# DeepMotionAIResearch/DenseMatchingBenchmark

Measured on AMD Instinct MI355X. Metric: stereo pairs/s (540x960, max_disp=192), higher is better.
Workload: dtype f32; 1 GPU; PSMNet Concatenation-volume + 3D aggregation + soft-argmin, 544x960 (540x960 padded), max_disp=192, batch 4 per GPU; costs_materialised=True, conv3d_mode=exact

## Files before the change

densematchingbenchmark_amd/_lib.py:

```python
import ctypes
import os
import re

import torch

_PKG = os.path.dirname(os.path.abspath(__file__))
DEV_BUILD = os.environ.get("DMB_LIB", "").startswith("dev")
LIB_PATH = os.path.join(_PKG, "lib", "libdmb_hip_%s.so" % os.environ["DMB_LIB"] if DEV_BUILD else "libdmb_hip.so")
DECONV3D_WORKSPACE_BYTES = 2048
CONV_SINGLE_CHAIN = 0x100
DEEPPRUNER_LOSS_WORKSPACE_DOUBLES = 9216
HEADER_PATH = os.path.join(os.path.dirname(_PKG), "include", "dmb_hip.h")

_c_int, _c_float, _c_void_p, _c_ll, _c_double = ctypes.c_int, ctypes.c_float, ctypes.c_void_p, ctypes.c_longlong, ctypes.c_double
_P = _c_void_p
_HI = ctypes.POINTER(ctypes.c_int)
_HF = ctypes.POINTER(ctypes.c_float)

ABI_VERSION = 8

SIGNATURES = {
    "dmb_abi_version": (_c_int, []),
    "dmb_last_error": (ctypes.c_char_p, []),
    "dmb_build_id": (ctypes.c_char_p, []),
    "dmb_cat_fms_f32": (_c_int, [_P, _P, _P, _c_int, _c_int, _c_int, _c_int, _c_int, _HI, _P]),
    "dmb_dif_fms_f32": (_c_int, [_P, _P, _P, _c_int, _c_int, _c_int, _c_int, _c_int, _HI, _P]),
    "dmb_gwc_fms_f32": (_c_int, [_P, _P, _P, _c_int, _c_int, _c_int, _c_int, _c_int, _c_int, _HI, _c_int, _c_int, _P]),
    "dmb_fast_cat_fms_f32": (_c_int, [_P, _P, _P, _P] + [_c_int] * 6 + [_P]),
    "dmb_fast_dif_fms_f32": (_c_int, [_P, _P, _P, _P] + [_c_int] * 7 + [_c_float, _P]),
    "dmb_fast_fms_bwd_f32": (_c_int, [_P] * 9 + [_c_int] * 7 + [_c_float, _P]),
    "dmb_spn_gaterecurrent2d_f32": (_c_int, [_P] * 5 + [_c_int] * 6 + [_P]),
    "dmb_spn_gaterecurrent2d_bwd_f32": (_c_int, [_P] * 10 + [_c_int] * 6 + [_P]),
    "dmb_conv2d_k3_multi_f32": (_c_int, [_c_int, _P, _P, _P, _P, _P, _c_int, _c_int, _c_int, _c_int, _P]),
    "dmb_cat_fms_into_f32": (_c_int, [_P, _P, _P, _c_int, _c_int, _c_int, _c_int, _c_int, _HI, _c_int, _c_int, _P]),
    "dmb_correlation1d_f32": (_c_int, [_P, _P, _P, _c_int, _c_int, _c_int, _c_int, _c_int, _c_float, _P]),
    "dmb_copy_window_f32": (_c_int, [_P, _P, _c_ll, _c_int, _c_int, _c_int, _P]),
    "dmb_catconv_pack_weights_f32": (_c_int, [_P, _P, _c_int, _c_int, _c_int, _c_int, _P]),
    "dmb_catconv_finalize_f32": (_c_int, [_P] * 8 + [_c_int] * 8 + [_P]),
    "dmb_catconv_combine_f32": (_c_int, [_P] * 9 + [_c_int] * 7 + [_P]),
    "dmb_conv3d_packed_floats": (_c_ll, [_c_int, _c_int]),
    "dmb_deconv3d_packed_floats": (_c_ll, [_c_int, _c_int]),
    "dmb_conv3d_pack_weights_f32": (_c_int, [_P, _P, _c_int, _c_int, _P]),
    "dmb_deconv3d_pack_weights_f32": (_c_int, [_P, _P, _c_int, _c_int, _P]),
    "dmb_conv3d_k3_f32": (_c_int, [_P, _P, _P, _P, _P, _P] + [_c_int] * 8 + [_P]),
    "dmb_conv3d_k3_c1_f32": (_c_int, [_P, _P, _c_float, _P, _P] + [_c_int] * 6 + [_P]),
    "dmb_deconv3d_k3s2_f32": (_c_int, [_P, _P, _P, _P, _P, _P] + [_c_int] * 8 + [_P, _P]),
    "dmb_conv3d_k3_hw_f32": (_c_int, [_P, _P, _P, _P, _P, _P] + [_c_int] * 8 + [_P]),
    "dmb_deconv3d_k3_hw_f32": (_c_int, [_P, _P, _P, _P, _P, _P] + [_c_int] * 7 + [_P]),
    "dmb_zero_columns_f32": (_c_int, [_P, _c_ll, _c_int, _c_int, _P]),
    "dmb_trilinear_ac_f32": (_c_int, [_P, _P] + [_c_int] * 7 + [_P]),
    "dmb_deconv3d_k8s4_c1_f32": (_c_int, [_P, _P, _P] + [_c_int] * 4 + [_P]),
    "dmb_deconv3d_k8s4_c1_soft_argmin_f32": (_c_int, [_P, _P, _P, _P] + [_c_int] * 4 + [_c_float, _HF, _P]),
    "dmb_soft_argmin_f32": (_c_int, [_P, _P, _c_int, _c_int, _c_int, _c_int, _c_float, _c_int, _HF, _P]),
    "dmb_soft_argmin_sampled_f32": (_c_int, [_P, _P, _P, _c_int, _c_int, _c_int, _c_int, _c_float, _c_int, _P]),
    "dmb_local_soft_argmin_f32": (_c_int, [_P, _P, _P] + [_c_int] * 8 + [_c_float, _P]),
    "dmb_trilinear_soft_argmin_f32": (_c_int, [_P, _P] + [_c_int] * 7 + [_c_float, _HF, _P]),
    "dmb_trilinear_ac_soft_argmin_f32": (_c_int, [_P, _P, _P] + [_c_int] * 7 + [_c_float, _HF, _P]),
    "dmb_conf_head_packed_floats": (_c_ll, [_c_int, _c_int]),
    "dmb_conf_head_pack_weights_f32": (_c_int, [_P, _P, _c_int, _c_int, _P]),
    "dmb_conf_head_f32": (_c_int, [_P, _P, _P, _P, _P, _P] + [_c_int] * 5 + [_P]),
    "dmb_conf_gather_f32": (_c_int, [_P, _P, _P] + [_c_int] * 4 + [_P]),
    "dmb_conf_phase_conv2d_f32": (_c_int, [_P] * 6 + [_c_int] * 5 + [_P]),
    "dmb_conf_ring_f32": (_c_int, [_P] * 6 + [_c_int] * 5 + [_P]),
    "dmb_conv2d_packed_floats": (_c_ll, [_c_int, _c_int, _c_int]),
    "dmb_conv2d_pack_weights_f32": (_c_int, [_P, _P, _c_int, _c_int, _c_int, _P]),
    "dmb_conv2d_f32": (_c_int, [_P, _P, _P, _P, _P, _P] + [_c_int] * 12 + [_P]),
    "dmb_avgpool2d_f32": (_c_int, [_P, _P] + [_c_int] * 7 + [_P]),
    "dmb_bilinear_ac_f32": (_c_int, [_P, _P] + [_c_int] * 8 + [_P]),
# ... 183 lines not shown
```

densematchingbenchmark_amd/csrc/conv3d.hip:

```cpp
#include <type_traits>

#include "dmb_common.h"

#ifndef DMB_S1_GSTR
#define DMB_S1_GSTR 1
#endif

#ifndef DMB_EPI_LD
#define DMB_EPI_LD 0
#endif
#ifndef DMB_EPI_ST
#define DMB_EPI_ST 0
#endif

namespace dmb {

__global__ void pack_weights_kernel(const float* __restrict__ w, float* __restrict__ wp, int Co, int Ci, int Cipad,
                                    int transposed) {
  const int NTT = cdiv(Co, 32);
  const long long total = (long long)Cipad * 27 * NTT * 32;
  for (long long i = blockIdx.x * (long long)blockDim.x + threadIdx.x; i < total; i += (long long)gridDim.x * blockDim.x) {
    const int lane = (int)(i & 63);
    long long r = i >> 6;
    const int nt = (int)(r % NTT);
// ... 27 lines not shown
    const int nt = (int)(r % NTT);
    r /= NTT;
    const int tap = (int)(r % 27);
    const int kp = (int)(r / 27);
    const int co = nt * 32 + (lane & 31);
    const int ci = 2 * kp + (lane >> 5);
    float v = 0.f;
    if (ci < Ci && co < Co)
      v = transposed == 2 ? jb.w[((size_t)ci * Co + co) * 27 + 26 - tap]
                          : (transposed ? jb.w[((size_t)ci * Co + co) * 27 + tap] : jb.w[((size_t)co * Ci + ci) * 27 + tap]);
    jb.wp[i] = v;
  }
}

struct Affine {
  const float* scale;
  const float* shift;
};

template <int CIN_, int COUT_, int TY_, int TX_, int CK_, int WN_, int SCHED_ = 1, int G_ = 0, int PMIN_ = 0, bool LIN_ = false>
struct S1Cfg {
  static constexpr int CIN = CIN_, COUT = COUT_, TY = TY_, TX = TX_, CK = CK_, WN = WN_, SCHED = SCHED_;
  static constexpr bool LIN = LIN_;
  static constexpr int G = G_;
  static constexpr bool ROWPAIR = G_ != 0;
  static constexpr int GR = G_ ? 32 / G_ : 1;
  static constexpr int WZ = 4 / WN;
  static constexpr int TZ = WZ;
  static constexpr int XOFF = ROWPAIR ? 3 : 0;
  static constexpr int PV = (4 + TX + 1 + 3) / 4 * 4;
  static constexpr int P = ROWPAIR ? (PV > PMIN_ ? PV : PMIN_) : TX + 2;
  static constexpr int ROWS = TY + 2;
  static constexpr int PLANE = ROWS * P;
  static constexpr int ZS = TZ + 2;
  static constexpr int UPR = P / 4, UPC = ZS * ROWS * UPR;
  static constexpr int IPC = (UPC + 63) / 64;
  static constexpr int TR_PITCH = 36;
  static constexpr int XS = ROWPAIR ? TX / (G_ ? G_ : 1) : 1;
  static constexpr int MT = LIN ? 2 : (ROWPAIR ? (TY / GR) * XS : (TY * P + 31) / 32);
  static constexpr int GSTR = (G_ == 16 && TY_ == 4 && !LIN_ && (2 * P) % 32 == 16 && P % 32 != 16 && DMB_S1_GSTR) ? 2 : 1;
  __device__ static constexpr int row_base(int q) { return GSTR == 2 ? q : GR * q; }
  __device__ static constexpr int lane_off(int j) { return ROWPAIR ? (j / (G_ ? G_ : 1)) * GSTR * P + (j % (G_ ? G_ : 1)) : j; }
  __device__ static constexpr int tile_off(int mt) { return ROWPAIR ? row_base(mt / XS) * P + (mt % XS) * G_ : mt * 32; }
  __device__ static void decode(int mt, int j, int& ly, int& lx, bool& valid) {
    if (ROWPAIR) {
      ly = row_base(mt / XS) + GSTR * (j / (G_ ? G_ : 1));
// ... 1 lines not shown
      valid = true;
    } else {
      const int m = mt * 32 + j;
      ly = m / P;
      lx = m - ly * P;
      valid = m < TY * P && lx < TX;
    }
  }
  static constexpr int NTT = COUT / 32;
  static constexpr int NT = NTT / WN;
  static constexpr int CH_STRIDE = ZS * PLANE + (ROWPAIR ? 4 : 36);
  static constexpr int NK = (CK / 2) * 27;
  static constexpr int IN_FLOATS = CK * CH_STRIDE;
  static constexpr int BUF_FLOATS = IN_FLOATS + NK * NTT * 64;
  static constexpr int LDS_FLOATS = 2 * BUF_FLOATS;
  static constexpr int WPE = (ROWPAIR && LDS_FLOATS * 4 * 3 <= 160 * 1024) ? 3 : 2;
  static_assert(ROWPAIR || P <= 64, "one wave stages one tile row per instruction");
  static_assert(CK % 2 == 0 && COUT % (32 * WN) == 0 && IN_FLOATS % 4 == 0, "shape");
  static_assert(!ROWPAIR || LIN || (G_ % 4 == 0 && TX % (G_ ? G_ : 1) == 0 && TY % GR == 0), "row-group tiles need TX % G == 0 and TY % (32 / G) == 0");
  static_assert(!LIN || (ROWPAIR && TY == 3 && TX % 4 == 0 && TX >= 32), "linear tiles: vector path, 3 + 2 staged rows, full-width rows");
  static_assert(!ROWPAIR || ((CK * IPC) % 4 == 0 && NT == 1 && LDS_FLOATS >= 4 * 32 * TR_PITCH), "row-pair staging / scratch");
};

template <int VEC>
__device__ __forceinline__ void store_tile(const f32x16 (&a)[VEC], const float (&sc)[16], const float (&sh)[16],
                                           const float* __restrict__ rb, float* __restrict__ yb, int co0, int h,
                                           unsigned cstride, unsigned o, int relu, int cvalid = 1 << 30) {
  float rv[16][VEC];
  if (rb) {
#pragma unroll
    for (int r = 0; r < 16; ++r) {
      if (co0 + cd_row(r, h) >= cvalid) {
        rv[r][0] = 0.f;
        rv[r][VEC - 1] = 0.f;
        continue;
      }
      const float* rp = rb + (size_t)(co0 + cd_row(r, h)) * cstride + o;
      if (VEC == 2) {
        const float2 t = *reinterpret_cast<const float2*>(rp);
        rv[r][0] = t.x;
        rv[r][VEC - 1] = t.y;
      } else {
        rv[r][0] = *rp;
      }
    }
  }
// ... 12 lines not shown
    if (VEC == 2)
      *reinterpret_cast<float2*>(yp) = make_float2(v[0], v[VEC - 1]);
    else
      *yp = v[0];
  }
}

template <class C, bool WITH_RES, bool STATS = false>
__global__ __launch_bounds__(256, C::WPE) void conv3d_s1_kernel(const float* __restrict__ x, const float* __restrict__ wp,
                                                           const float* __restrict__ scale,
                                                           const float* __restrict__ shift,
                                                           const float* __restrict__ res, float* __restrict__ y, int Ci,
                                                           int D, int H, int W, int ntx, int nty, int ntz, int relu,
                                                           double* __restrict__ stats) {
  extern __shared__ __attribute__((aligned(16))) float lds[];
  const int dbg = DMB_DBG((relu >> 8) & 0xff);
  const int stg = DMB_DBG(relu >> 16);
  relu &= 0xff;
  if (stg > 0 && blockIdx.x < 256u * C::WPE) {
    const int n = (int)(__builtin_amdgcn_s_getreg((3 << 11) | (16 << 6) | 4) & 15u) * stg;
    for (int i = 0; i < n; ++i) __builtin_amdgcn_s_sleep(127);
  }
  int t = xcd_remap(blockIdx.x, gridDim.x);
  const int tx = t % ntx;
  t /= ntx;
  const int ty = t % nty;
  t /= nty;
  const int tz = t % ntz;
  const int b = t / ntz;
  const int p0 = C::LIN ? tx * 64 : 0;
  const int x0 = C::LIN ? 0 : tx * C::TX, y0 = C::LIN ? p0 / W : ty * C::TY, z0 = tz * C::TZ;

  const int wave = __builtin_amdgcn_readfirstlane(threadIdx.x >> 6), lane = threadIdx.x & 63;
  const int j = lane & 31, h = lane >> 5;
  const int wz = wave / C::WN, wn = wave % C::WN;
  const unsigned HW = (unsigned)H * W, DHW = (unsigned)D * HW;
  const float* xb = x + (size_t)b * Ci * DHW;

  f32x16 acc[C::MT][C::NT];

  constexpr int NPL = C::CK * C::ZS;
  static_assert(NPL % 4 == 0, "planes are dealt evenly to the 4 waves");
  constexpr int PPW = NPL / 4;
  constexpr int WCH = C::NK * C::NTT * 64;
  static_assert(WCH % 16 == 0, "weights are staged with 16-byte copies, evenly over 4 waves");
  constexpr int WPW = WCH / 16;
// ... 69 lines not shown
#pragma unroll
    for (int ks = 0; ks < C::NK; ++ks) {
      if (ks + 1 < C::NK) load_frag(ks + 1, af[(ks + 1) & 1], bf[(ks + 1) & 1]);
      if (C::SCHED != 0) __builtin_amdgcn_sched_barrier(0);
#pragma unroll
      for (int mt = 0; mt < C::MT; ++mt)
#pragma unroll
        for (int nt = 0; nt < C::NT; ++nt) {
          if (FIRST && ks == 0) {
            const f32x16 zero = {0.f, 0.f, 0.f, 0.f, 0.f, 0.f, 0.f, 0.f, 0.f, 0.f, 0.f, 0.f, 0.f, 0.f, 0.f, 0.f};
            acc[mt][nt] = DMB_MFMA(af[0][nt], bf[0][mt], zero);
          } else {
            acc[mt][nt] = DMB_MFMA(af[ks & 1][nt], bf[ks & 1][mt], acc[mt][nt]);
          }
        }
      if (C::SCHED != 0) __builtin_amdgcn_sched_barrier(0);
    }
    if (!(dbg & 32)) __syncthreads();
  };
  chunk(std::true_type{}, 0);
  for (int ci = 1; ci < NC; ++ci) chunk(std::false_type{}, ci);

  if (dbg & 1) return;
  const int gz = z0 + wz;
  float* yb = y + (size_t)b * C::COUT * DHW;
  const float* rb = res ? res + (size_t)b * C::COUT * DHW : nullptr;
  if constexpr (C::ROWPAIR) {
    float* my = lds + wave * (32 * C::TR_PITCH);
    const __amdgpu_buffer_rsrc_t yrs = make_rsrc(yb, (unsigned)C::COUT * DHW * 4u);
    const __amdgpu_buffer_rsrc_t rrs = make_rsrc(rb ? rb : yb, (unsigned)C::COUT * DHW * 4u);
    const int px = (lane & 7) * 4;
    const float lo = relu == 1 ? 0.f : -__builtin_inff();
    const float lo2 = relu == 2 ? 0.f : -__builtin_inff();
    float sc4[4], sh4[4];
#pragma unroll
    for (int k = 0; k < 4; ++k) {
      const int co = wn * 32 + k * 8 + (lane >> 3);
      sc4[k] = scale ? scale[co] : 1.f;
      sh4[k] = shift ? shift[co] : 0.f;
    }
    const unsigned kstep = 8u * DHW * 4u;
    auto offset0 = [&](int mt) {
      if constexpr (C::LIN) {
        const unsigned pos = (unsigned)(p0 + mt * 32 + px);
        return (gz < D && pos < HW) ? ((unsigned)(wn * 32 + (lane >> 3)) * DHW + (unsigned)gz * HW + pos) * 4u : DMA_OOB;
      }
// ... 1091 lines not shown
      }
  __syncthreads();
  const int q = wave, oz = q >> 1, oy = q & 1;
  float v[4];
#pragma unroll
  for (int i = 0; i < 4; ++i) {
    float s = tiles[(q * 4 + i) * 64 + lane];
#pragma unroll
    for (int ww = 1; ww < 4; ++ww) s += tiles[ww * C1S_TILE + (q * 4 + i) * 64 + lane];
    v[i] = s + bias;
  }
  const int gx = x0 - 4 + lq * 4, gz = z0 + oz, gy = y0 + 2 * lyp + oy;
  if (lq == 0 || gx >= W || gz >= D || gy >= H) return;
  const size_t o = (size_t)b * DHW + (size_t)gz * HW + (size_t)gy * W + gx;
  float4 r4 = make_float4(v[0], v[1], v[2], v[3]);
  if (res) {
    const float4 r = *reinterpret_cast<const float4*>(res + o);
    r4.x += r.x; r4.y += r.y; r4.z += r.z; r4.w += r.w;
  }
  *reinterpret_cast<float4*>(y + o) = r4;
}


static long long cdiv_ll(long long a, long long b) { return (a + b - 1) / b; }
template <class C>
static int launch_s1(const float* x, const float* wp, const float* scale, const float* shift, const float* res,
                     float* y, int B, int Ci, int D, int H, int W, int relu, hipStream_t st) {
  const int ntx = C::LIN ? cdiv(H * W, 64) : cdiv(W, C::TX), nty = C::LIN ? 1 : cdiv(H, C::TY), ntz = cdiv(D, C::TZ);
  const long long nblk = (long long)B * ntx * nty * ntz;
  if (nblk > 0x7fffffffLL) return fail(DMB_EUNSUPPORTED, "conv3d: grid too large");
  const size_t lds = (size_t)C::LDS_FLOATS * sizeof(float) + (size_t)DMB_OPT(17) * 1024;
  if (DMB_OPT(17)) {
    (void)hipFuncSetAttribute(reinterpret_cast<const void*>(&conv3d_s1_kernel<C, true>), hipFuncAttributeMaxDynamicSharedMemorySize, (int)lds);
    (void)hipFuncSetAttribute(reinterpret_cast<const void*>(&conv3d_s1_kernel<C, false>), hipFuncAttributeMaxDynamicSharedMemorySize, (int)lds);
  }
  if (res) {
    DMB_ENSURE_LDS((&conv3d_s1_kernel<C, true>), (size_t)(lds));
    hipLaunchKernelGGL((conv3d_s1_kernel<C, true>), dim3((unsigned)nblk), dim3(256), lds, st, x, wp, scale, shift, res, y, Ci, D,
                       H, W, ntx, nty, ntz, relu, (double*)nullptr);
  } else {
    DMB_ENSURE_LDS((&conv3d_s1_kernel<C, false>), (size_t)(lds));
    hipLaunchKernelGGL((conv3d_s1_kernel<C, false>), dim3((unsigned)nblk), dim3(256), lds, st, x, wp, scale, shift, res, y, Ci, D,
                       H, W, ntx, nty, ntz, relu, (double*)nullptr);
  }
  return launch_status("conv3d stride-1 launch failed");
}
// ... 242 lines not shown

static bool s1_stats_applicable(const float* x, const float* y, int B, int Ci, int Co, int D, int H, int W) {
  return Co == 32 && Ci > 0 && W % 4 == 0 && (((uintptr_t)x | (uintptr_t)y) & 15) == 0 && (long long)Co * D * H * W * 4 < 0x7fffffffLL &&
         (long long)8 * D * H * W * 4 < 0x7fffffffLL && DMB_OPT(2) == 0;
}
extern "C" long long dmb_conv3d_k3_bnstats_partials(int B, int Ci, int Co, int D, int H, int W) {
  if (B <= 0 || D <= 0 || H <= 0 || W <= 0 || Co != 32 || Ci <= 0 || W % 4 != 0) return 0;
  if ((long long)Co * D * H * W * 4 >= 0x7fffffffLL || (long long)8 * D * H * W * 4 >= 0x7fffffffLL) return 0;
  return s1_blocks32(s1_pick32(B, D, H, W), B, D, H, W);
}
extern "C" int dmb_conv3d_k3_bnstats_f32(const float* x, const float* wpack, float* y, double* stats, int B, int Ci, int Co, int D, int H,
                                         int W, void* stream) {
  if (!x || !wpack || !y || !stats || B <= 0 || Ci <= 0 || D <= 0 || H <= 0 || W <= 0) return fail(DMB_EINVAL, "conv3d_bnstats: bad argument");
  if (!s1_stats_applicable(x, y, B, Ci, Co, D, H, W)) return fail(DMB_EUNSUPPORTED, "conv3d_bnstats: 32 output channels, 16-byte rows");
  hipStream_t st = (hipStream_t)stream;
  switch (s1_pick32(B, D, H, W)) {
    case 0: return launch_s1_stats<S1Cfg<0, 32, 4, 48, 2, 1, 1, 16, 0>>(x, wpack, y, stats, B, Ci, D, H, W, st);
    case 1: return launch_s1_stats<S1Cfg<0, 32, 8, 24, 2, 1, 1, 8, 40>>(x, wpack, y, stats, B, Ci, D, H, W, st);
    case 2: return launch_s1_stats<S1Cfg<0, 32, 4, 32, 2, 1, 1, 16, 0>>(x, wpack, y, stats, B, Ci, D, H, W, st);
    default: return launch_s1_stats<S1Cfg<0, 32, 2, 32, 2, 1, 1, 16, 0>>(x, wpack, y, stats, B, Ci, D, H, W, st);
  }
}

static int dsk_variant(int B, int Ci, int Co, int D, int H, int W) {
  const long long tiles = (long long)B * D * cdiv(H, 2) * cdiv(W, 16);
  const int ncu = num_cus();
  const long long units = tiles * cdiv(Co, 32);
  if (Ci % 8 == 0 && Ci <= 64 && units <= 5LL * ncu) return 3;
  return 0;
}

extern "C" int dmb_deconv3d_k3s2_f32(const float* x, const float* wpack, const float* scale, const float* shift,
                                     const float* residual, float* y, int B, int Ci, int Co, int D, int H, int W, int Wout,
                                     int relu, void* workspace, void* stream) {
  if (!x || !wpack || !y || B <= 0 || Ci <= 0 || D <= 0 || H <= 0 || W <= 0) return fail(DMB_EINVAL, "deconv3d: bad argument");
  if (Wout <= 0 || Wout > 2 * W || Wout <= 2 * W - 8 || (Wout & 1)) return fail(DMB_EINVAL, "deconv3d: Wout must be 2 W, or 2 W minus the (at most 3) doubled padding columns");
  if ((long long)8 * D * H * W * 4 >= 0x7fffffffLL)
    return fail(DMB_EUNSUPPORTED, "deconv3d: 8 input channels of one batch item must stay below 2 GiB (32-bit buffer offsets)");
  hipStream_t st = (hipStream_t)stream;
  const bool single_chain = (relu & DMB_CONV_SINGLE_CHAIN) != 0;
  relu &= 0xff;
  relu |= DMB_OPT(6) << 8;
  {
    int v = single_chain ? 0 : dsk_variant(B, Ci, Co, D, H, W);
    if (DMB_OPT(25) == 1) v = 0;
    if (DMB_OPT(25) >= 2) v = DMB_OPT(25) - 1;
// ... 51 lines not shown
```

densematchingbenchmark_amd/csrc/torch_shim.cpp:

```cpp
#include <torch/extension.h>

#include <c10/hip/HIPStream.h>

#include <string>
#include <tuple>
#include <vector>

#include "dmb_hip.h"

namespace {

PyObject* g_error_class = nullptr;

[[noreturn]] void raise(const std::string& msg) {
  PyErr_SetString(g_error_class ? g_error_class : PyExc_RuntimeError, msg.c_str());
  throw py::error_already_set();
}

void chk(int rc, const char* what) {
  if (rc != DMB_OK) raise(std::string(what) + " failed with code " + std::to_string(rc) + " (" + dmb_last_error() + ")");
}

const at::Tensor& f32(const at::Tensor& t, const char* name) {
  if (!t.is_cuda())
// ... 52 lines not shown
  void* ws = nullptr;
  if (workspace.has_value()) {
    const at::Tensor& w = *workspace;
    if (!w.is_cuda() || w.scalar_type() != at::kInt || !w.is_contiguous() || w.numel() * 4 < DMB_DECONV3D_WORKSPACE_BYTES || w.device() != x.device())
      raise("deconv3d_k3s2: workspace must be a contiguous int32 tensor of DMB_DECONV3D_WORKSPACE_BYTES on the input's device");
    ws = w.data_ptr();
  }
  chk(dmb_deconv3d_k3s2_f32(ptr(x, "x"), ptr(wpack, "wpack"), optr(scale, "scale"), optr(shift, "shift"), optr(residual, "residual"),
                            y.data_ptr<float>(), (int)B, (int)Ci, (int)Co, (int)D, (int)H, (int)W, (int)Wout, (int)relu_flags, ws, stream_of(x)),
      "dmb_deconv3d_k3s2_f32");
  return y;
}

at::Tensor conv3d_k3_c1(const at::Tensor& x, const at::Tensor& w, double bias, const c10::optional<at::Tensor>& residual, int64_t flags) {
  f32(x, "x");
  if (x.dim() != 5) raise("conv3d_k3_c1: x must be [B, Ci, D, H, W]");
  const int64_t B = x.size(0), Ci = x.size(1), D = x.size(2), H = x.size(3), W = x.size(4);
  if (w.numel() != Ci * 27) raise("conv3d_k3_c1: weight does not belong to this channel count");
  at::Tensor y = at::empty({B, 1, D, H, W}, x.options());
  if (residual.has_value() && residual->sizes() != y.sizes()) raise("conv3d_k3_c1 residual: shapes differ");
  chk(dmb_conv3d_k3_c1_f32(ptr(x, "x"), ptr(w, "weight"), (float)bias, optr(residual, "residual"), y.data_ptr<float>(), (int)B, (int)Ci,
                           (int)D, (int)H, (int)W, (int)flags, stream_of(x)),
      "dmb_conv3d_k3_c1_f32");
  return y;
}

std::vector<at::Tensor> trilinear_ac_soft_argmin(const at::Tensor& x, int64_t Do, int64_t Ho, int64_t Wo, double alpha,
                                                 const std::vector<float>& disp_values) {
  f32(x, "x");
  if (x.dim() != 4) raise("trilinear_ac_soft_argmin: x must be [B, D, H, W]");
  if ((int64_t)disp_values.size() != Do) raise("trilinear_ac_soft_argmin: one disparity sample value per output plane");
  const int64_t B = x.size(0);
  at::Tensor y = at::empty({B, Do, Ho, Wo}, x.options()), disp = at::empty({B, 1, Ho, Wo}, x.options());
  chk(dmb_trilinear_ac_soft_argmin_f32(ptr(x, "x"), y.data_ptr<float>(), disp.data_ptr<float>(), (int)B, (int)x.size(1), (int)x.size(2),
                                       (int)x.size(3), (int)Do, (int)Ho, (int)Wo, (float)alpha, disp_values.data(), stream_of(x)),
      "dmb_trilinear_ac_soft_argmin_f32");
  return {y, disp};
}

at::Tensor conv2d(const at::Tensor& x, int64_t coff, int64_t Ci, const at::Tensor& wpack, int64_t Co, int64_t ksize, int64_t stride,
                  int64_t dilation, const c10::optional<at::Tensor>& scale, const c10::optional<at::Tensor>& shift,
                  const c10::optional<at::Tensor>& residual, int64_t res_off, int64_t relu_flags, const c10::optional<at::Tensor>& out,
                  int64_t out_off) {
  f32(x, "x");
  if (x.dim() != 4) raise("conv2d: x must be [B, C, H, W]");
  const int64_t B = x.size(0), Cx = x.size(1), H = x.size(2), W = x.size(3);
// ... 119 lines not shown
}

void set_error_class(py::object cls) {
  Py_XDECREF(g_error_class);
  g_error_class = cls.ptr();
  Py_XINCREF(g_error_class);
}

}

#ifndef DMB_SHIM_ID
#define DMB_SHIM_ID "unknown"
#endif

PYBIND11_MODULE(TORCH_EXTENSION_NAME, m) {
  m.doc() = "thin torch extension over libdmb_hip.so's C ABI (include/dmb_hip.h): unwrap tensors, current HIP stream, raise on error";
  m.def("set_error_class", &set_error_class);
  m.def("build_id", []() { return std::string(DMB_SHIM_ID); });
  m.def("library_build_id", []() { return std::string(dmb_build_id()); });
  m.def("abi_version", []() { return dmb_abi_version(); });
  m.def("conv3d_k3", &conv3d_k3);
  m.def("deconv3d_k3s2", &deconv3d_k3s2);
  m.def("conv3d_k3_c1", &conv3d_k3_c1);
  m.def("trilinear_ac_soft_argmin", &trilinear_ac_soft_argmin);
  m.def("conv2d", &conv2d);
  m.def("copy_window", &copy_window);
  m.def("bn_train_fwd", &bn_train_fwd);
  m.def("bn_act_bwd", &bn_act_bwd);
  m.def("conv2d_wgrad", &conv2d_wgrad);
}
```

densematchingbenchmark_amd/modeling/stereo/cost_processors/aggregators/PSMNet.py:

```python
import torch
import torch.nn as nn

from ..... import ops
from ...layers import train_fn
from ...layers.basic_layers import HeadConv3d, conv3d_bn, conv3d_bn_relu
from ..utils.hourglass import Hourglass


class PSMAggregator(nn.Module):

    accepts_lazy_cat = True

    def __init__(self, max_disp, in_planes=64, batch_norm=True):
        super().__init__()
        self.max_disp, self.in_planes, self.batch_norm = max_disp, in_planes, batch_norm
        bn = batch_norm
        self.dres0 = nn.Sequential(conv3d_bn_relu(bn, in_planes, 32, 3, 1, 1, bias=False),
                                   conv3d_bn_relu(bn, 32, 32, 3, 1, 1, bias=False))
        self.dres1 = nn.Sequential(conv3d_bn_relu(bn, 32, 32, 3, 1, 1, bias=False),
                                   conv3d_bn(bn, 32, 32, 3, 1, 1, bias=False))
        self.dres2 = Hourglass(in_planes=32, batch_norm=bn)
        self.dres3 = Hourglass(in_planes=32, batch_norm=bn)
        self.dres4 = Hourglass(in_planes=32, batch_norm=bn)
        self.classif1 = nn.Sequential(conv3d_bn_relu(bn, 32, 32, 3, 1, 1, bias=False), HeadConv3d(32, bias=False))
        self.classif2 = nn.Sequential(conv3d_bn_relu(bn, 32, 32, 3, 1, 1, bias=False), HeadConv3d(32, bias=False))
        self.classif3 = nn.Sequential(conv3d_bn_relu(bn, 32, 32, 3, 1, 1, bias=False), HeadConv3d(32, bias=False))

    def trunk(self, raw_cost):
        cost0 = self.dres0(raw_cost)
        cost0 = self.dres1[1](self.dres1[0](cost0), residual=cost0)
        out1, pre1, post1 = self.dres2(cost0, None, None, skip=cost0)
        out2, pre2, post2 = self.dres3(out1, pre1, post1, skip=cost0)
        out3, pre3, post3 = self.dres4(out2, pre2, post2, skip=cost0)
        cost1 = self.classif1[1](self.classif1[0](out1))
        cost2 = self.classif2[1](self.classif2[0](out2), residual=cost1)
        cost3 = self.classif3[1](self.classif3[0](out3), residual=cost2)
        return cost1, cost2, cost3

    def _forward_overlapped(self, raw_cost):
        B, C, D, H, W = raw_cost.shape
        size = (self.max_disp, H * 4, W * 4)
        vals = ops.disp_sample_values(self.max_disp, 0, 1)
        main = torch.cuda.current_stream(raw_cost.device)
        side = ops.side_stream(raw_cost.device)

        def upsample(c):
            cost, disp = ops.trilinear_ac_soft_argmin(c.squeeze(1), size, vals, 1.0)
            cost.record_stream(main)
            disp.record_stream(main)
            return ops.RegressionHint.attach(cost, vals, 1.0, disp)

        cost0 = self.dres0(raw_cost)
        cost0 = self.dres1[1](self.dres1[0](cost0), residual=cost0)
        out1, pre1, post1 = self.dres2(cost0, None, None, skip=cost0)
        fork1 = main.record_event()
        with torch.cuda.stream(side):
            side.wait_event(fork1)
            cost1 = self.classif1[1](self.classif1[0](out1))
            up1 = upsample(cost1)
        out2, pre2, post2 = self.dres3(out1, pre1, post1, skip=cost0)
        fork2 = main.record_event()
        with torch.cuda.stream(side):
            side.wait_event(fork2)
            cost2 = self.classif2[1](self.classif2[0](out2), residual=cost1)
            cost2.record_stream(main)
            join2 = side.record_event()
            up2 = upsample(cost2)
            done = side.record_event()
        out3, pre3, post3 = self.dres4(out2, pre2, post2, skip=cost0)
        main.wait_event(join2)
        cost3 = self.classif3[1](self.classif3[0](out3), residual=cost2)
        up3 = upsample(cost3)
        main.wait_event(done)
        return [up3, up2, up1]

    def forward(self, raw_cost):
        B, C, D, H, W = raw_cost.shape
        if ops.branch_overlap(raw_cost) and raw_cost.device.type == "cuda" and not train_fn.wants_grad(self, raw_cost):
            return self._forward_overlapped(raw_cost)
        with train_fn.carry_scope():
            cost1, cost2, cost3 = self.trunk(raw_cost)
        size = (self.max_disp, H * 4, W * 4)
        vals = ops.disp_sample_values(self.max_disp, 0, 1)
        up = []
        for c in (cost3, cost2, cost1):
            if train_fn.wants_grad(self, c):
                cost, disp = train_fn.UpsampleRegressFn.apply(c.squeeze(1), size, tuple(vals), 1.0)
            else:
                cost, disp = ops.trilinear_ac_soft_argmin(c.squeeze(1), size, vals, 1.0)
            up.append(ops.RegressionHint.attach(cost, vals, 1.0, disp))
        return up
```

densematchingbenchmark_amd/modeling/stereo/layers/basic_layers.py:

```python
import torch
import torch.nn as nn

from .... import ops, param_state
from . import train_fn

__all__ = ["FusedConv3d", "HeadConv3d", "HeadDeconv3d", "conv3d_bn", "conv3d_bn_relu", "deconv3d_bn", "deconv3d_bn_relu",
           "bn_parts", "fold_batch_norm"]


def fold_batch_norm(bn, conv_bias, out_planes, device):
    if bn is None:
        if conv_bias is None:
            return None, None
        return torch.ones(out_planes, dtype=torch.float32, device=device), conv_bias.detach().float().contiguous()
    if bn.running_mean is None or bn.running_var is None:
        raise NotImplementedError("fold_batch_norm: a BatchNorm without running statistics (track_running_stats=False) "
                                  "normalises with batch statistics in eval() too; it has no folded form")
    var = bn.running_var.detach().double()
    mean = bn.running_mean.detach().double()
    gamma = bn.weight.detach().double() if bn.affine else torch.ones_like(var)
    beta = bn.bias.detach().double() if bn.affine else torch.zeros_like(var)
    scale = gamma / torch.sqrt(var + bn.eps)
    shift = beta - mean * scale
    if conv_bias is not None:
        shift = shift + conv_bias.detach().double() * scale
    return scale.float().contiguous(), shift.float().contiguous()


def bn_parts(bn):
    return () if bn is None else (bn.weight, bn.bias, bn.running_mean, bn.running_var, bn.num_batches_tracked)
# ... 123 lines not shown

class HeadConv3d(nn.Conv3d):

    def __init__(self, in_planes, bias=False):
        super().__init__(in_planes, 1, kernel_size=3, stride=1, padding=1, bias=bias)

    def train(self, mode=True):
        epoch_on_mode_switch(self, mode)
        return super().train(mode)

    def forward(self, x, residual=None):
        if hasattr(x, "materialize"):
            x = x.materialize()
        if train_fn.wants_grad(self, x, residual):
            return train_fn.HeadConvFn.apply(x, self.weight, self.bias, residual)
        return ops.conv3d_k3_c1(x, self.weight.detach(), self.bias_value(), residual)

    def bias_value(self):
        if self.bias is None:
            return 0.0
        return param_state.cached(self, "_dmb_bias", (self.bias,), lambda: float(self.bias.detach().cpu()[0]))


class HeadDeconv3d(nn.ConvTranspose3d):

    def __init__(self, in_planes, out_planes):
        super().__init__(in_planes, out_planes, kernel_size=3, stride=2, padding=1, output_padding=1)

    def forward(self, x):
        if train_fn.wants_grad(self, x):
            return train_fn.HeadDeconvFn.apply(x, self.weight, self.bias)
        wp, bias = param_state.cached(self, "_dmb_packed", (self.weight, self.bias), lambda: (
            ops.pack_deconv3d_weights(self.weight.detach()), self.bias.detach().float().contiguous()))
        return ops.deconv3d_k3s2(x, wp, self.out_channels, None, bias, None, False)


def conv3d_bn(batchNorm, in_planes, out_planes, kernel_size=3, stride=1, padding=1, dilation=1, bias=True):
    return FusedConv3d(batchNorm, in_planes, out_planes, kernel_size, stride, padding, dilation, bias, relu=False)


def conv3d_bn_relu(batchNorm, in_planes, out_planes, kernel_size=3, stride=1, padding=1, dilation=1, bias=True):
    return FusedConv3d(batchNorm, in_planes, out_planes, kernel_size, stride, padding, dilation, bias, relu=True)


def deconv3d_bn(batchNorm, in_planes, out_planes, kernel_size=4, stride=2, padding=1, output_padding=0, bias=True):
    return FusedConv3d(batchNorm, in_planes, out_planes, kernel_size, stride, padding, 1, bias, relu=False,
# ... 7 lines not shown
```

include/dmb_hip.h:

```cpp
#ifndef DMB_HIP_H
#define DMB_HIP_H

#ifdef __cplusplus
extern "C" {
#endif

#define DMB_OK 0
#define DMB_EINVAL 100001
#define DMB_EUNSUPPORTED 100002

#define DMB_MAX_DISP_SAMPLES 256

int dmb_abi_version(void);
const char* dmb_last_error(void);
const char* dmb_build_id(void);


int dmb_cat_fms_f32(const float* L, const float* R, float* out, int B, int C, int H, int W, int D,
                    const int* disp_idx_host, void* stream);

int dmb_dif_fms_f32(const float* L, const float* R, float* out, int B, int C, int H, int W, int D,
                    const int* disp_idx_host, void* stream);

int dmb_fast_cat_fms_f32(const float* L, const float* R, const float* disp_sample, float* out, int B, int C, int D, int H,
// ... 24 lines not shown
                            const float* GB, const float* scale, const float* shift, float* out, int B, int Co, int CA, int D,
                            int H, int W, int relu, void* stream);

int dmb_correlation1d_f32(const float* L, const float* R, float* out, int B, int C, int H, int W, int D,
                          float negative_slope, void* stream);

int dmb_cat_fms_into_f32(const float* L, const float* R, float* out, int B, int C, int H, int W, int D,
                         const int* disp_idx_host, int out_channels, int out_ch_offset, void* stream);

#define DMB_CONV_SINGLE_CHAIN 0x100

long long dmb_conv3d_packed_floats(int Co, int Ci);
long long dmb_deconv3d_packed_floats(int Ci, int Co);

int dmb_conv3d_pack_weights_f32(const float* w, float* wpack, int Co, int Ci, void* stream);
int dmb_deconv3d_pack_weights_f32(const float* w, float* wpack, int Ci, int Co, void* stream);

int dmb_conv3d_k3_f32(const float* x, const float* wpack, const float* scale, const float* shift,
                      const float* residual, float* y, int B, int Ci, int Co, int D, int H, int W,
                      int stride, int relu, void* stream);

int dmb_conv3d_k3_c1_f32(const float* x, const float* w, float bias, const float* residual, float* y,
                         int B, int Ci, int D, int H, int W, int flags, void* stream);

#define DMB_DECONV3D_WORKSPACE_BYTES 2048
int dmb_deconv3d_k3s2_f32(const float* x, const float* wpack, const float* scale, const float* shift,
                          const float* residual, float* y, int B, int Ci, int Co, int D, int H, int W, int Wout,
                          int relu, void* workspace, void* stream);

int dmb_conv3d_k3_hw_f32(const float* x, const float* wpack, const float* scale, const float* shift,
                         const float* residual, float* y, int B, int Ci, int Co, int D, int H, int W,
                         int stride_hw, int relu, void* stream);

int dmb_deconv3d_k3_hw_f32(const float* x, const float* wpack, const float* scale, const float* shift,
                           const float* residual, float* y, int B, int Ci, int Co, int D, int H, int W, int relu,
                           void* stream);


int dmb_trilinear_ac_f32(const float* x, float* y, int B, int Di, int Hi, int Wi, int Do, int Ho, int Wo,
                         void* stream);

int dmb_deconv3d_k8s4_c1_f32(const float* x, const float* w, float* y, int B, int D, int H, int W,
                             void* stream);

int dmb_deconv3d_k8s4_c1_soft_argmin_f32(const float* x, const float* w, float* y, float* disp, int B, int D, int H, int W,
                                         float alpha, const float* disp_sample_host, void* stream);
// ... 229 lines not shown
```

Baseline: 149.9 pairs/s.

## Fuse classifier conv3d 32-channel layer with single-channel head conv

Adds a fused kernel for the classifier branches. The 32-channel 3x3x3 conv with BN and ReLU is followed in the same block by a 32->1 3x3x3 head conv done via MFMA. Each tile writes partial sums for its halo-extended output to a workspace, and a finish kernel sums overlapping tile contributions and adds bias and residual. This avoids writing and re-reading the 32-channel intermediate volume and one full conv launch, at the cost of extra halo workspace traffic, a second launch and LDS scatter work.

```diff
diff --git a/densematchingbenchmark_amd/_lib.py b/densematchingbenchmark_amd/_lib.py
--- a/densematchingbenchmark_amd/_lib.py
+++ b/densematchingbenchmark_amd/_lib.py
@@ -9,6 +9,7 @@
 LIB_PATH = os.path.join(_PKG, "lib", "libdmb_hip_%s.so" % os.environ["DMB_LIB"] if DEV_BUILD else "libdmb_hip.so")
 DECONV3D_WORKSPACE_BYTES = 2048
 CONV_SINGLE_CHAIN = 0x100
+CONV3D_HEAD_PACKED_FLOATS = 1024
 DEEPPRUNER_LOSS_WORKSPACE_DOUBLES = 9216
 HEADER_PATH = os.path.join(os.path.dirname(_PKG), "include", "dmb_hip.h")
 
@@ -44,6 +45,10 @@
     "dmb_deconv3d_pack_weights_f32": (_c_int, [_P, _P, _c_int, _c_int, _P]),
     "dmb_conv3d_k3_f32": (_c_int, [_P, _P, _P, _P, _P, _P] + [_c_int] * 8 + [_P]),
     "dmb_conv3d_k3_c1_f32": (_c_int, [_P, _P, _c_float, _P, _P] + [_c_int] * 6 + [_P]),
+    "dmb_conv3d_k3_head_workspace_floats": (_c_ll, [_c_int] * 4),
+    "dmb_conv3d_k3_head_preferred": (_c_int, [_c_int] * 4),
+    "dmb_conv3d_head_pack_weights_f32": (_c_int, [_P, _P, _P]),
+    "dmb_conv3d_k3_head_f32": (_c_int, [_P] * 5 + [_c_float, _P, _P, _P] + [_c_int] * 6 + [_P]),
     "dmb_deconv3d_k3s2_f32": (_c_int, [_P, _P, _P, _P, _P, _P] + [_c_int] * 8 + [_P, _P]),
     "dmb_conv3d_k3_hw_f32": (_c_int, [_P, _P, _P, _P, _P, _P] + [_c_int] * 8 + [_P]),
     "dmb_deconv3d_k3_hw_f32": (_c_int, [_P, _P, _P, _P, _P, _P] + [_c_int] * 7 + [_P]),
diff --git a/densematchingbenchmark_amd/csrc/conv3d.hip b/densematchingbenchmark_amd/csrc/conv3d.hip
--- a/densematchingbenchmark_amd/csrc/conv3d.hip
+++ b/densematchingbenchmark_amd/csrc/conv3d.hip
@@ -73,6 +73,7 @@
 struct S1Cfg {
   static constexpr int CIN = CIN_, COUT = COUT_, TY = TY_, TX = TX_, CK = CK_, WN = WN_, SCHED = SCHED_;
   static constexpr bool LIN = LIN_;
+  static constexpr bool HEAD = false;
   static constexpr int G = G_;
   static constexpr bool ROWPAIR = G_ != 0;
   static constexpr int GR = G_ ? 32 / G_ : 1;
@@ -120,6 +121,17 @@
   static_assert(!ROWPAIR || ((CK * IPC) % 4 == 0 && NT == 1 && LDS_FLOATS >= 4 * 32 * TR_PITCH), "row-pair staging / scratch");
 };
 
+struct S1HeadCfg : S1Cfg<0, 32, 4, 48, 2, 1, 1, 16, 0> {
+  static constexpr bool HEAD = true;
+  static constexpr int OZ = TZ + 2, OY = TY + 2, OX = TX + 2;
+  static constexpr int OUT_FLOATS = OZ * OY * OX;
+  static constexpr int OP = 56, OPLANE = OY * OP;
+  static_assert(GSTR == 2 && XS == 3 && MT == 6 && OX % 2 == 0 && OX <= OP && (2 * OP) % 32 == 16, "head tile");
+  static_assert(OZ * OPLANE + 64 <= LDS_FLOATS && (OZ * OPLANE) % 4 == 0, "the partial-sum tile lives in the freed chunk buffers");
+};
+constexpr int HEAD_PACKED_FLOATS = 16 * 64;
+static_assert(HEAD_PACKED_FLOATS == DMB_CONV3D_HEAD_PACKED_FLOATS, "include/dmb_hip.h");
+
 template <int VEC>
 __device__ __forceinline__ void store_tile(const f32x16 (&a)[VEC], const float (&sc)[16], const float (&sh)[16],
                                            const float* __restrict__ rb, float* __restrict__ yb, int co0, int h,
@@ -178,6 +190,7 @@
     for (int i = 0; i < n; ++i) __builtin_amdgcn_s_sleep(127);
   }
   int t = xcd_remap(blockIdx.x, gridDim.x);
+  const int tile = t;
   const int tx = t % ntx;
   t /= ntx;
   const int ty = t % nty;
@@ -293,6 +306,75 @@
   for (int ci = 1; ci < NC; ++ci) chunk(std::false_type{}, ci);
 
   if (dbg & 1) return;
+  if constexpr (C::HEAD) {
+    float* ot = lds;
+    float* tab = lds + C::OZ * C::OPLANE;
+    float aw[16];
+#pragma unroll
+    for (int s = 0; s < 16; ++s) aw[s] = res[s * 64 + lane];
+    for (int i = threadIdx.x; i < C::OZ * C::OPLANE / 4; i += 256) reinterpret_cast<float4*>(ot)[i] = make_float4(0.f, 0.f, 0.f, 0.f);
+    if (threadIdx.x < 32) {
+      const int co = cd_row(threadIdx.x & 15, threadIdx.x >> 4);
+      tab[threadIdx.x * 2] = scale ? scale[co] : 1.f;
+      tab[threadIdx.x * 2 + 1] = shift ? shift[co] : 0.f;
+    }
+    __syncthreads();
+    const float lo = relu ? 0.f : -__builtin_inff();
+#pragma unroll
+    for (int r = 0; r < 16; ++r) {
+      const float2 ss = *reinterpret_cast<const float2*>(tab + (h * 16 + r) * 2);
+#pragma unroll
+      for (int mt = 0; mt < C::MT; ++mt) acc[mt][0][r] = fmaxf(fmaf(acc[mt][0][r], ss.x, ss.y), lo);
+    }
+#pragma unroll
+    for (int mt = 0; mt < C::MT; ++mt) {
+      const f32x16 zero = {0.f, 0.f, 0.f, 0.f, 0.f, 0.f, 0.f, 0.f, 0.f, 0.f, 0.f, 0.f, 0.f, 0.f, 0.f, 0.f};
+      f32x16 p = DMB_MFMA(aw[0], acc[mt][0][0], zero);
+#pragma unroll
+      for (int s = 1; s < 16; ++s) p = DMB_MFMA(aw[s], acc[mt][0][s], p);
+      acc[mt][0] = p;
+    }
+#pragma unroll
+    for (int mt = 0; mt < C::MT; ++mt) {
+      const int gy = y0 + C::row_base(mt / C::XS) + C::GSTR * (j >> 4), gxo = x0 + (mt % C::XS) * 16 + (j & 15);
+      const bool inb = z0 + wz < D && gy < H && gxo < W;
+#pragma unroll
+      for (int r = 0; r < 16; ++r) acc[mt][0][r] = inb ? acc[mt][0][r] : 0.f;
+    }
+    float* ob = ot + (wz * C::OY + C::GSTR * (j >> 4)) * C::OP + (j & 15);
+#pragma unroll
+    for (int dz = 0; dz < 3; ++dz) {
+      if (dz) __syncthreads();
+#pragma unroll
+      for (int hh = 0; hh < 2; ++hh) {
+        if (h != hh) continue;
+#pragma unroll
+        for (int r = 0; r < 16; ++r) {
+          const int tap = cd_row(r, hh);
+          if (tap >= 27 || tap / 9 != dz) continue;
+          float cur[C::MT];
+#pragma unroll
+          for (int mt = 0; mt < C::MT; ++mt) {
+            const int o0 = ((2 - dz) * C::OY + C::row_base(mt / C::XS) + 2) * C::OP + (mt % C::XS) * 16 + 2;
+            cur[mt] = ob[o0 - ((tap / 3) % 3) * C::OP - tap % 3];
+          }
+#pragma unroll
+          for (int mt = 0; mt < C::MT; ++mt) {
+            const int o0 = ((2 - dz) * C::OY + C::row_base(mt / C::XS) + 2) * C::OP + (mt % C::XS) * 16 + 2;
+            ob[o0 - ((tap / 3) % 3) * C::OP - tap % 3] = cur[mt] + acc[mt][0][r];
+          }
+          asm volatile("" ::: "memory");
+        }
+      }
+    }
+    __syncthreads();
+    float* wt = y + (size_t)tile * C::OUT_FLOATS;
+    for (int i = threadIdx.x; i < C::OUT_FLOATS / 2; i += 256) {
+      const int rw = i / (C::OX / 2), c2 = i - rw * (C::OX / 2);
+      *reinterpret_cast<float2*>(wt + rw * C::OX + c2 * 2) = *reinterpret_cast<const float2*>(ot + rw * C::OP + c2 * 2);
+    }
+    return;
+  }
   const int gz = z0 + wz;
   float* yb = y + (size_t)b * C::COUT * DHW;
   const float* rb = res ? res + (size_t)b * C::COUT * DHW : nullptr;
@@ -1430,6 +1512,49 @@
 }
 
 
+__global__ void pack_head_weights_kernel(const float* __restrict__ w, float* __restrict__ whp) {
+  const int i = blockIdx.x * blockDim.x + threadIdx.x;
+  if (i >= HEAD_PACKED_FLOATS) return;
+  const int lane = i & 63, s = i >> 6, tap = lane & 31;
+  whp[i] = tap < 27 ? w[cd_row(s, lane >> 5) * 27 + tap] : 0.f;
+}
+
+__global__ __launch_bounds__(256) void conv3d_head_finish_kernel(const float* __restrict__ ws, const float* __restrict__ res,
+                                                                 float* __restrict__ y, float bias, int D, int H, int W, int ntx,
+                                                                 int nty, int ntz, long long total) {
+  using C = S1HeadCfg;
+  const long long idx = (long long)blockIdx.x * 256 + threadIdx.x;
+  if (idx >= total) return;
+  const int gx = (int)(idx % W);
+  long long q = idx / W;
+  const int gy = (int)(q % H);
+  q /= H;
+  const int gz = (int)(q % D), b = (int)(q / D);
+  const int tz = gz / C::TZ, ty = gy / C::TY, tx = gx / C::TX;
+  const int lz = gz - tz * C::TZ, ly = gy - ty * C::TY, lx = gx - tx * C::TX;
+  float s = 0.f;
+  bool any = false;
+  for (int a = -1; a <= 1; ++a) {
+    const int oz = lz - a * C::TZ + 1;
+    if (oz < 0 || oz >= C::OZ || tz + a < 0 || tz + a >= ntz) continue;
+    for (int c = -1; c <= 1; ++c) {
+      const int oy = ly - c * C::TY + 1;
+      if (oy < 0 || oy >= C::OY || ty + c < 0 || ty + c >= nty) continue;
+      for (int e = -1; e <= 1; ++e) {
+        const int ox = lx - e * C::TX + 1;
+        if (ox < 0 || ox >= C::OX || tx + e < 0 || tx + e >= ntx) continue;
+        const size_t slot = (((size_t)b * ntz + (tz + a)) * nty + (ty + c)) * ntx + (tx + e);
+        const float v = ws[slot * C::OUT_FLOATS + (oz * C::OY + oy) * C::OX + ox];
+        s = any ? s + v : v;
+        any = true;
+      }
+    }
+  }
+  s += bias;
+  if (res) s += res[idx];
+  y[idx] = s;
+}
+
 static long long cdiv_ll(long long a, long long b) { return (a + b - 1) / b; }
 template <class C>
 static int launch_s1(const float* x, const float* wp, const float* scale, const float* shift, const float* res,
@@ -1718,6 +1843,47 @@
   }
 }
 
+static bool s1_head_runs(int B, int D, int H, int W) {
+  if (B <= 0 || D <= 0 || H <= 0 || W <= 0 || W % 4 != 0 || DMB_OPT(2) != 0) return false;
+  return (long long)32 * D * H * W * 4 < 0x7fffffffLL;
+}
+extern "C" long long dmb_conv3d_k3_head_workspace_floats(int B, int D, int H, int W) {
+  if (!s1_head_runs(B, D, H, W)) return 0;
+  return s1_blocks32(0, B, D, H, W) * S1HeadCfg::OUT_FLOATS;
+}
+extern "C" int dmb_conv3d_k3_head_preferred(int B, int D, int H, int W) {
+  return s1_head_runs(B, D, H, W) && s1_pick32(B, D, H, W) == 0;
+}
+extern "C" int dmb_conv3d_head_pack_weights_f32(const float* w, float* wpack, void* stream) {
+  if (!w || !wpack) return fail(DMB_EINVAL, "conv3d_head_pack_weights: bad argument");
+  hipLaunchKernelGGL(pack_head_weights_kernel, dim3(HEAD_PACKED_FLOATS / 256), dim3(256), 0, (hipStream_t)stream, w, wpack);
+  return launch_status("conv3d_head_pack_weights launch failed");
+}
+extern "C" int dmb_conv3d_k3_head_f32(const float* x, const float* wpack, const float* scale, const float* shift,
+                                      const float* head_wpack, float bias, const float* residual, float* y, float* workspace,
+                                      int B, int Ci, int D, int H, int W, int relu, void* stream) {
+  using C = S1HeadCfg;
+  if (!x || !wpack || !head_wpack || !y || !workspace || B <= 0 || Ci <= 0 || D <= 0 || H <= 0 || W <= 0)
+    return fail(DMB_EINVAL, "conv3d_head: bad argument");
+  if (relu & DMB_CONV_SINGLE_CHAIN) return fail(DMB_EUNSUPPORTED, "conv3d_head: not a single-chain sum (use dmb_conv3d_k3_f32 + dmb_conv3d_k3_c1_f32)");
+  relu &= 0xff;
+  if (!s1_head_runs(B, D, H, W) || (((uintptr_t)x) & 15) != 0 || (((uintptr_t)workspace) & 7) != 0)
+    return fail(DMB_EUNSUPPORTED, "conv3d_head: 16-byte rows only (W % 4 == 0, x 16-byte aligned, 32 channels of one batch item below 2 GiB), workspace 8-byte aligned");
+  hipStream_t st = (hipStream_t)stream;
+  const int ntx = cdiv(W, C::TX), nty = cdiv(H, C::TY), ntz = cdiv(D, C::TZ);
+  const long long nblk = (long long)B * ntx * nty * ntz, total = (long long)B * D * H * W;
+  if (nblk > 0x7fffffffLL || cdiv_ll(total, 256) > 0x7fffffffLL) return fail(DMB_EUNSUPPORTED, "conv3d_head: grid too large");
+  const size_t lds = (size_t)C::LDS_FLOATS * sizeof(float);
+  DMB_ENSURE_LDS((&conv3d_s1_kernel<C, false>), (size_t)(lds));
+  hipLaunchKernelGGL((conv3d_s1_kernel<C, false>), dim3((unsigned)nblk), dim3(256), lds, st, x, wpack, scale, shift, head_wpack,
+                     workspace, Ci, D, H, W, ntx, nty, ntz, relu, (double*)nullptr);
+  const int rc = launch_status("conv3d_head launch failed");
+  if (rc != DMB_OK) return rc;
+  hipLaunchKernelGGL(conv3d_head_finish_kernel, dim3((unsigned)cdiv_ll(total, 256)), dim3(256), 0, st, workspace, residual, y, bias, D,
+                     H, W, ntx, nty, ntz, total);
+  return launch_status("conv3d_head finishing launch failed");
+}
+
 static int dsk_variant(int B, int Ci, int Co, int D, int H, int W) {
   const long long tiles = (long long)B * D * cdiv(H, 2) * cdiv(W, 16);
   const int ncu = num_cus();
diff --git a/densematchingbenchmark_amd/csrc/torch_shim.cpp b/densematchingbenchmark_amd/csrc/torch_shim.cpp
--- a/densematchingbenchmark_amd/csrc/torch_shim.cpp
+++ b/densematchingbenchmark_amd/csrc/torch_shim.cpp
@@ -98,6 +98,27 @@
   chk(dmb_conv3d_k3_c1_f32(ptr(x, "x"), ptr(w, "weight"), (float)bias, optr(residual, "residual"), y.data_ptr<float>(), (int)B, (int)Ci,
                            (int)D, (int)H, (int)W, (int)flags, stream_of(x)),
       "dmb_conv3d_k3_c1_f32");
+  return y;
+}
+
+at::Tensor conv3d_k3_head(const at::Tensor& x, const at::Tensor& wpack, const c10::optional<at::Tensor>& scale,
+                          const c10::optional<at::Tensor>& shift, const at::Tensor& head_wpack, double bias,
+                          const c10::optional<at::Tensor>& residual, int64_t relu_flags) {
+  f32(x, "x");
+  if (x.dim() != 5) raise("conv3d_k3_head: x must be [B, Ci, D, H, W]");
+  const int64_t B = x.size(0), Ci = x.size(1), D = x.size(2), H = x.size(3), W = x.size(4);
+  affine_ok(scale, shift, 32, "conv3d_k3_head");
+  if (wpack.numel() != dmb_conv3d_packed_floats(32, (int)Ci)) raise("conv3d_k3_head: packed weights do not belong to these channel counts");
+  if (head_wpack.numel() != DMB_CONV3D_HEAD_PACKED_FLOATS) raise("conv3d_k3_head: head weights must come from conv3d_head_pack_weights");
+  const long long wsf = dmb_conv3d_k3_head_workspace_floats((int)B, (int)D, (int)H, (int)W);
+  if (wsf <= 0) raise("conv3d_k3_head: this shape does not take the fused form (use conv3d_k3 + conv3d_k3_c1)");
+  at::Tensor y = at::empty({B, 1, D, H, W}, x.options());
+  if (residual.has_value() && residual->sizes() != y.sizes()) raise("conv3d_k3_head residual: shapes differ");
+  at::Tensor ws = at::empty({(int64_t)wsf}, x.options());
+  chk(dmb_conv3d_k3_head_f32(ptr(x, "x"), ptr(wpack, "wpack"), optr(scale, "scale"), optr(shift, "shift"), ptr(head_wpack, "head_wpack"),
+                             (float)bias, optr(residual, "residual"), y.data_ptr<float>(), ws.data_ptr<float>(), (int)B, (int)Ci, (int)D,
+                             (int)H, (int)W, (int)relu_flags, stream_of(x)),
+      "dmb_conv3d_k3_head_f32");
   return y;
 }
 
@@ -263,6 +284,7 @@
   m.def("conv3d_k3", &conv3d_k3);
   m.def("deconv3d_k3s2", &deconv3d_k3s2);
   m.def("conv3d_k3_c1", &conv3d_k3_c1);
+  m.def("conv3d_k3_head", &conv3d_k3_head);
   m.def("trilinear_ac_soft_argmin", &trilinear_ac_soft_argmin);
   m.def("conv2d", &conv2d);
   m.def("copy_window", &copy_window);
diff --git a/densematchingbenchmark_amd/modeling/stereo/cost_processors/aggregators/PSMNet.py b/densematchingbenchmark_amd/modeling/stereo/cost_processors/aggregators/PSMNet.py
--- a/densematchingbenchmark_amd/modeling/stereo/cost_processors/aggregators/PSMNet.py
+++ b/densematchingbenchmark_amd/modeling/stereo/cost_processors/aggregators/PSMNet.py
@@ -3,7 +3,7 @@
 
 from ..... import ops
 from ...layers import train_fn
-from ...layers.basic_layers import HeadConv3d, conv3d_bn, conv3d_bn_relu
+from ...layers.basic_layers import HeadConv3d, classifier_branch, conv3d_bn, conv3d_bn_relu
 from ..utils.hourglass import Hourglass
 
 
@@ -32,9 +32,9 @@
         out1, pre1, post1 = self.dres2(cost0, None, None, skip=cost0)
         out2, pre2, post2 = self.dres3(out1, pre1, post1, skip=cost0)
         out3, pre3, post3 = self.dres4(out2, pre2, post2, skip=cost0)
-        cost1 = self.classif1[1](self.classif1[0](out1))
-        cost2 = self.classif2[1](self.classif2[0](out2), residual=cost1)
-        cost3 = self.classif3[1](self.classif3[0](out3), residual=cost2)
+        cost1 = classifier_branch(self.classif1[0], self.classif1[1], out1)
+        cost2 = classifier_branch(self.classif2[0], self.classif2[1], out2, cost1)
+        cost3 = classifier_branch(self.classif3[0], self.classif3[1], out3, cost2)
         return cost1, cost2, cost3
 
     def _forward_overlapped(self, raw_cost):
@@ -56,20 +56,20 @@
         fork1 = main.record_event()
         with torch.cuda.stream(side):
             side.wait_event(fork1)
-            cost1 = self.classif1[1](self.classif1[0](out1))
+            cost1 = classifier_branch(self.classif1[0], self.classif1[1], out1)
             up1 = upsample(cost1)
         out2, pre2, post2 = self.dres3(out1, pre1, post1, skip=cost0)
         fork2 = main.record_event()
         with torch.cuda.stream(side):
             side.wait_event(fork2)
-            cost2 = self.classif2[1](self.classif2[0](out2), residual=cost1)
+            cost2 = classifier_branch(self.classif2[0], self.classif2[1], out2, cost1)
             cost2.record_stream(main)
             join2 = side.record_event()
             up2 = upsample(cost2)
             done = side.record_event()
         out3, pre3, post3 = self.dres4(out2, pre2, post2, skip=cost0)
         main.wait_event(join2)
-        cost3 = self.classif3[1](self.classif3[0](out3), residual=cost2)
+        cost3 = classifier_branch(self.classif3[0], self.classif3[1], out3, cost2)
         up3 = upsample(cost3)
         main.wait_event(done)
         return [up3, up2, up1]
diff --git a/densematchingbenchmark_amd/modeling/stereo/layers/basic_layers.py b/densematchingbenchmark_amd/modeling/stereo/layers/basic_layers.py
--- a/densematchingbenchmark_amd/modeling/stereo/layers/basic_layers.py
+++ b/densematchingbenchmark_amd/modeling/stereo/layers/basic_layers.py
@@ -1,11 +1,11 @@
 import torch
 import torch.nn as nn
 
-from .... import ops, param_state
+from .... import ops, ops_head, param_state
 from . import train_fn
 
 __all__ = ["FusedConv3d", "HeadConv3d", "HeadDeconv3d", "conv3d_bn", "conv3d_bn_relu", "deconv3d_bn", "deconv3d_bn_relu",
-           "bn_parts", "fold_batch_norm"]
+           "bn_parts", "classifier_branch", "fold_batch_norm"]
 
 
 def fold_batch_norm(bn, conv_bias, out_planes, device):
@@ -175,6 +175,17 @@
         return param_state.cached(self, "_dmb_bias", (self.bias,), lambda: float(self.bias.detach().cpu()[0]))
 
 
+def classifier_branch(unit, head, x, residual=None):
+    if (isinstance(unit, FusedConv3d) and isinstance(head, HeadConv3d) and torch.is_tensor(x) and x.dim() == 5
+            and unit.out_planes == 32 and head.in_channels == 32 and unit.stride == 1 and not unit.transposed and unit.has_relu
+            and not train_fn.wants_grad(unit, x) and not train_fn.wants_grad(head, x, residual)
+            and ops_head.conv3d_k3_head_applicable(x)):
+        wp, scale, shift = unit._prepacked()
+        hw = param_state.cached(head, "_dmb_packed_head", (head.weight,), lambda: ops_head.pack_conv3d_head_weights(head.weight.detach()))
+        return ops_head.conv3d_k3_head(x, wp, hw, scale, shift, head.bias_value(), residual, True)
+    return head(unit(x), residual=residual)
+
+
 class HeadDeconv3d(nn.ConvTranspose3d):
 
     def __init__(self, in_planes, out_planes):
diff --git a/densematchingbenchmark_amd/ops_head.py b/densematchingbenchmark_amd/ops_head.py
--- /dev/null
+++ b/densematchingbenchmark_amd/ops_head.py
@@ -0,0 +1,55 @@
+import torch
+
+from . import _lib, ops
+from .ops import _affine_ok, _f32c, _relu_mode, _same_shape, check, dev_ptr, stream_ptr
+
+
+def pack_conv3d_head_weights(w):
+    lib = _lib.load()
+    w = _f32c(w, "weight")
+    if tuple(w.shape) != (1, 32, 3, 3, 3):
+        raise _lib.DmbLibraryError("pack_conv3d_head_weights: weight must be [1, 32, 3, 3, 3], got %s" % (tuple(w.shape),))
+    wp = torch.empty((_lib.CONV3D_HEAD_PACKED_FLOATS,), dtype=torch.float32, device=w.device)
+    check(lib.dmb_conv3d_head_pack_weights_f32(dev_ptr(w), dev_ptr(wp), stream_ptr(w.device)), "dmb_conv3d_head_pack_weights_f32")
+    return wp
+
+
+def conv3d_k3_head_applicable(x):
+    if x.dim() != 5 or x.dtype != torch.float32 or x.device.type != "cuda" or not ops.split_k() or ops.conv3d_mode() != "exact":
+        return False
+    B, _, D, H, W = x.shape
+    return x.data_ptr() % 16 == 0 and _lib.load().dmb_conv3d_k3_head_preferred(B, D, H, W) == 1
+
+
+def conv3d_k3_head(x, wpack, head_wpack, scale=None, shift=None, bias=0.0, residual=None, relu=True):
+    tag = "conv3d_k3_head_%dto32to1" % x.shape[1]
+    sh = _lib.shim()
+    if sh is not None:
+        if ops._kernel_timer is not None:
+            ops._kernel_timer.start(tag)
+        y = sh.conv3d_k3_head(x if x.is_contiguous() else x.contiguous(), wpack, scale, shift, head_wpack, float(bias), residual,
+                              _relu_mode(relu) | ops._conv_flags())
+        if ops._kernel_timer is not None:
+            ops._kernel_timer.stop(tag)
+        return y
+    lib = _lib.load()
+    x = _f32c(x, "x")
+    B, Ci, D, H, W = x.shape
+    _affine_ok(scale, shift, 32, "conv3d_k3_head")
+    if wpack.numel() != lib.dmb_conv3d_packed_floats(32, Ci) or head_wpack.numel() != _lib.CONV3D_HEAD_PACKED_FLOATS:
+        raise _lib.DmbLibraryError("conv3d_k3_head: packed weights do not belong to %d -> 32 -> 1 channels" % Ci)
+    wsf = lib.dmb_conv3d_k3_head_workspace_floats(B, D, H, W)
+    if wsf <= 0:
+        raise _lib.DmbLibraryError("conv3d_k3_head: shape %s does not take the fused form (use conv3d_k3 + conv3d_k3_c1)" % (tuple(x.shape),))
+    y = torch.empty((B, 1, D, H, W), dtype=torch.float32, device=x.device)
+    if residual is not None:
+        _same_shape(residual, y, "conv3d_k3_head residual")
+    ws = torch.empty((wsf,), dtype=torch.float32, device=x.device)
+    if ops._kernel_timer is not None:
+        ops._kernel_timer.start(tag)
+    check(lib.dmb_conv3d_k3_head_f32(dev_ptr(x), dev_ptr(wpack), dev_ptr(scale, allow_none=True), dev_ptr(shift, allow_none=True),
+                                     dev_ptr(head_wpack), float(bias), dev_ptr(residual, allow_none=True), dev_ptr(y), dev_ptr(ws),
+                                     B, Ci, D, H, W, _relu_mode(relu) | ops._conv_flags(), stream_ptr(x.device)), "dmb_conv3d_k3_head_f32")
+    if ops._kernel_timer is not None:
+        ops._kernel_timer.stop(tag)
+    return y
diff --git a/include/dmb_hip.h b/include/dmb_hip.h
--- a/include/dmb_hip.h
+++ b/include/dmb_hip.h
@@ -70,6 +70,14 @@
 
 int dmb_conv3d_k3_c1_f32(const float* x, const float* w, float bias, const float* residual, float* y,
                          int B, int Ci, int D, int H, int W, int flags, void* stream);
+
+#define DMB_CONV3D_HEAD_PACKED_FLOATS 1024
+long long dmb_conv3d_k3_head_workspace_floats(int B, int D, int H, int W);
+int dmb_conv3d_k3_head_preferred(int B, int D, int H, int W);
+int dmb_conv3d_head_pack_weights_f32(const float* w_head, float* head_wpack, void* stream);
+int dmb_conv3d_k3_head_f32(const float* x, const float* wpack, const float* scale, const float* shift,
+                           const float* head_wpack, float bias, const float* residual, float* y, float* workspace,
+                           int B, int Ci, int D, int H, int W, int relu, void* stream);
 
 #define DMB_DECONV3D_WORKSPACE_BYTES 2048
 int dmb_deconv3d_k3s2_f32(const float* x, const float* wpack, const float* scale, const float* shift,
```

Result: faster. 152.1 pairs/s (median of 6 runs) (+1.5%).
